# oswsnqc/Tensorflow-DPPO

Measured on AMD Instinct MI355X. Metric: env-steps/sec (whole node), Humanoid-shaped MLP DPPO at 1/2/4/8 MI355X, higher is better.
Workload: dtype fp32; 1 GPU; model=Humanoid-v4 MLP 64x64 tanh, preset=humanoid, global_batch=16777216, num_envs_per_gpu=262144, rollout_T=64, update_steps=4, parallelism=dp1

## Files before the change

dppo_amd/ops/hip/bindings.cpp:

```cpp
#include <torch/extension.h>

#include <vector>

std::vector<torch::Tensor> gae_scan(torch::Tensor rewards, torch::Tensor values,
                                    torch::Tensor dones, torch::Tensor boot,
                                    double gamma, double lam, bool whiten,
                                    double eps, torch::Tensor adv_out,
                                    torch::Tensor etr_out);

torch::Tensor ppo_loss_gauss_fwd(torch::Tensor pdpi, torch::Tensor pdold,
                                 torch::Tensor vpred, torch::Tensor oldv,
                                 torch::Tensor act, torch::Tensor adv,
                                 torch::Tensor etr, double clip,
                                 double entcoeff, double vcoeff);

torch::Tensor ppo_loss_gauss_gh(torch::Tensor pdflat, torch::Tensor oldflat,
                                torch::Tensor vpred, torch::Tensor oldv,
                                torch::Tensor act, torch::Tensor adv,
                                torch::Tensor etr, double clip,
                                double entcoeff, double vcoeff,
                                torch::Tensor clip_dev);

std::vector<torch::Tensor> ppo_loss_gauss_bwd(
    torch::Tensor pdpi, torch::Tensor pdold, torch::Tensor vpred,
// ... 35 lines not shown
                   torch::Tensor adv, torch::Tensor etr, torch::Tensor gh,
                   torch::Tensor clip_dev, double clip, double entcoeff,
                   double vcoeff);

void adam_step(torch::Tensor p, torch::Tensor g, torch::Tensor m,
               torch::Tensor v, int64_t step, double lr, double beta1,
               double beta2, double eps);

void adam_step_dev(torch::Tensor p, torch::Tensor g, torch::Tensor m,
                   torch::Tensor v, torch::Tensor step_dev,
                   torch::Tensor lr_dev, torch::Tensor coef, double beta1,
                   double beta2, double eps);

void gemm_fwd(torch::Tensor X, torch::Tensor Wt, torch::Tensor bias,
              int64_t activation, int64_t heads, torch::Tensor C,
              torch::Tensor v, torch::Tensor aux, int64_t wt_layout,
              int64_t ablate, int64_t ldc);

void dw_mfma(torch::Tensor delta, torch::Tensor acts, torch::Tensor grad_buf,
             int64_t w_off, int64_t b_off, int64_t split_row, int64_t w_off2,
             int64_t b_off2, int64_t ablate);

void rollout_sample(torch::Tensor pdflat, torch::Tensor actions,
                    torch::Tensor xva, torch::Tensor seed_dev,
                    torch::Tensor eps_dev, int64_t step, int64_t va_off,
                    double act_low, double act_high);

void gemm_env_step(torch::Tensor xva, torch::Tensor M, torch::Tensor xin,
                   torch::Tensor xout, torch::Tensor envd,
                   torch::Tensor horizons, torch::Tensor t,
                   torch::Tensor epr,
                   torch::Tensor rewards, torch::Tensor dones,
                   torch::Tensor rsum, torch::Tensor seed_dev, double sigma,
                   int64_t step);

void rollout_env_step(torch::Tensor xin, torch::Tensor xout, torch::Tensor G,
                      torch::Tensor envd, torch::Tensor horizons,
                      torch::Tensor t, torch::Tensor epr,
                      torch::Tensor rewards, torch::Tensor dones,
                      torch::Tensor seed_dev, double sigma, int64_t step);

torch::Tensor rollout_moments(torch::Tensor rewards, torch::Tensor dones,
                              torch::Tensor epr_in, int64_t T, int64_t E);

bool mlp_chunk_supported(int64_t D, int64_t H, int64_t A, int64_t n_hidden);

void mlp_chunk_train(
    torch::Tensor params, torch::Tensor states, torch::Tensor actions,
    torch::Tensor adv, torch::Tensor etr, torch::Tensor oldflat,
    torch::Tensor oldv, std::vector<int64_t> offsets,
    std::vector<int64_t> dims, int64_t activation, torch::Tensor clip_dev,
    double clip, double entcoeff, double vcoeff, torch::Tensor slabs,
    torch::Tensor mom, torch::Tensor vel, torch::Tensor step_dev,
    torch::Tensor lr_dev, torch::Tensor coef, torch::Tensor flat_grad,
    bool fuse_adam, double beta1, double beta2, double eps);

std::vector<torch::Tensor> rollout_run(
    torch::Tensor params, std::vector<int64_t> offsets,
    std::vector<int64_t> dims, int64_t activation,
    torch::Tensor envblob, int64_t rank, torch::Tensor horizons,
    double noise, double act_low, double act_high, double eps_explore,
    torch::Tensor x, torch::Tensor t, torch::Tensor epr,
    int64_t T, int64_t act_dim, int64_t seed, torch::Tensor out_buf,
    int64_t ablate);

PYBIND11_MODULE(TORCH_EXTENSION_NAME, mod) {
  mod.def("gae_scan", &gae_scan,
          "segmented GAE reverse scan + whitening (gfx950)");
  mod.def("ppo_loss_gauss_fwd", &ppo_loss_gauss_fwd,
          "fused DiagGaussian PPO loss forward (gfx950)");
  mod.def("ppo_loss_gauss_bwd", &ppo_loss_gauss_bwd,
          "fused DiagGaussian PPO loss backward (gfx950)");
  mod.def("ppo_loss_cat_fwd", &ppo_loss_cat_fwd,
          "fused Categorical PPO loss forward (gfx950)");
  mod.def("ppo_loss_cat_bwd", &ppo_loss_cat_bwd,
          "fused Categorical PPO loss backward (gfx950)");
  mod.def("cat_sample", &cat_sample,
          "Gumbel-max categorical sampling, counter-based RNG (gfx950)");
  mod.def("bf16_mm256", &bf16_mm256,
          "bf16 MFMA GEMM, 256^2 tile, pipelined glds, fused epilogues "
          "(gfx950)");
  mod.def("bf16_mm_small", &bf16_mm_small,
          "guarded bf16 MFMA GEMM for ragged heads shapes (gfx950)");
  mod.def("bf16_transpose", &bf16_transpose,
          "bf16 2D transpose with fused column sums (gfx950)");
  mod.def("gauss_gh_wide", &gauss_gh_wide,
          "wide-policy PPO loss gradient -> bf16 [g_pd | g_v] (gfx950)");
  mod.def("adam_step", &adam_step, "fused flat Adam step (gfx950)");
  mod.def("adam_step_dev", &adam_step_dev,
          "graph-replayable fused Adam (device step/lr) (gfx950)");
  mod.def("rollout_run", &rollout_run,
          "fused T-step rollout: MLP fwd + sample + synthetic env (gfx950)");
  mod.def("rollout_sample", &rollout_sample,
          "per-step action sampling + eps-greedy (v3 rollout) (gfx950)");
  mod.def("gemm_env_step", &gemm_env_step,
          "fused G-GEMM + env transition epilogue + per-env finish "
          "(v3 rollout; gfx950)");
  mod.def("rollout_env_step", &rollout_env_step,
          "per-step synthetic env finish: tanh/reward/done/reset (gfx950)");
  mod.def("rollout_moments", &rollout_moments,
          "episode-reward moments from reward/done streams (gfx950)");
  mod.def("ppo_loss_gauss_gh", &ppo_loss_gauss_gh,
          "wave-per-row PPO loss gradient -> [g_pd | g_v] (gfx950)");
  mod.def("gemm_fwd", &gemm_fwd,
          "MFMA f32 layer forward C=act(X@Wt+b), fused tanh (gfx950)");
  mod.def("dw_mfma", &dw_mfma,
          "MFMA f32 split-K dW += delta^T@acts into flat grad (gfx950)");
  mod.def("mlp_chunk_supported", &mlp_chunk_supported,
          "shape eligibility for the fused chunk-step kernel (gfx950)");
  mod.def("mlp_chunk_train", &mlp_chunk_train,
          "fused small-MLP training chunk step: fwd+PPO grad+bwd+dW "
          "partials + slab-reduce Adam (gfx950)");
}
```

dppo_amd/ops/hip/common.h:

```cpp
#pragma once

#include <hip/hip_runtime.h>

#define DEV_INLINE __device__ __forceinline__

constexpr int WAVE = 64;
constexpr int N_CU = 256;

DEV_INLINE float wave_reduce_sum(float x) {
  #pragma unroll
  for (int off = WAVE / 2; off > 0; off >>= 1) x += __shfl_down(x, off, WAVE);
  return x;
}

DEV_INLINE void wave_atomic_add(double* dst, float val) {
  float w = wave_reduce_sum(val);
  if ((threadIdx.x & (WAVE - 1)) == 0) atomicAdd(dst, static_cast<double>(w));
}

DEV_INLINE float fast_tanhf(float x) {
  const float e = __expf(2.0f * x);
  return 1.0f - 2.0f / (e + 1.0f);
}

DEV_INLINE int64_t gidx() {
  return static_cast<int64_t>(blockIdx.x) * blockDim.x + threadIdx.x;
}

DEV_INLINE int64_t gstride() {
  return static_cast<int64_t>(gridDim.x) * blockDim.x;
}

inline int elementwise_grid(int64_t n, int block) {
  int64_t g = (n + block - 1) / block;
  const int64_t cap = 2048;
  return static_cast<int>(g < cap ? (g > 0 ? g : 1) : cap);
}
```

dppo_amd/ops/hip/mfma_gemm.hip:

```cpp

#include <hip/hip_runtime.h>
#include <torch/extension.h>
#include <c10/hip/HIPStream.h>

#include "common.h"

namespace {

using f32x16 = __attribute__((ext_vector_type(16))) float;

constexpr int BK = 16;
constexpr int M_WAVE = 32;
constexpr int FWD_WAVES = 4;
constexpr int FWD_M = FWD_WAVES * M_WAVE;
constexpr int MAX_NT = 4;

DEV_INLINE int cd_row(int reg, int lane) {
  return (reg & 3) + 8 * (reg >> 2) + 4 * (lane >> 5);
}


struct FwdArgs {
  const float* X;
  const float* Wt;
  const float* bias;
  const float* aux;
  float* C;
  float* v;
  int64_t B;
  int K, N;
  int activation;
  int heads;
  int wt_layout;
  int ldc;
  int ablate;
  const float* env_xin;
  float* env_x;
  const float* envd;
  const int* horizons;
  const int* tcount;
  const long long* seed_dev;
  float* env_rsum;
  float sigma;
  int step;
};

DEV_INLINE unsigned g_lowbias32(unsigned x) {
  x ^= x >> 16;
  x *= 0x7feb352dU;
  x ^= x >> 15;
  x *= 0x846ca68bU;
  x ^= x >> 16;
  return x;
}
DEV_INLINE float2 g_rng_normal2(unsigned seed, int env, int step, int slot) {
  const unsigned h = g_lowbias32(seed ^ (unsigned)env * 0x9E3779B9U ^
                                 (unsigned)step * 0x85EBCA6BU ^
                                 (unsigned)slot * 0xC2B2AE35U);
  const float u1 = ((h >> 16) + 1) * (1.0f / 65537.0f);
  const float u2 = (h & 0xFFFFu) * (1.0f / 65536.0f);
  const float r = sqrtf(-2.0f * __logf(u1));
  float sn, cs;
  __sincosf(6.2831853071795865f * u2, &sn, &cs);
  return make_float2(r * cs, r * sn);
}
DEV_INLINE float g_rng_normal(unsigned seed, int env, int step, int slot) {
  return g_rng_normal2(seed, env, step, slot).x;
}

template <int NT>
__launch_bounds__(FWD_WAVES * 64)
__global__ void gemm_fwd_kernel(FwdArgs a) {
  const int lane = threadIdx.x & (WAVE - 1);
  const int wave = threadIdx.x / WAVE;

// ... 266 lines not shown
      if (col < a.N) {
        const float bv = (a.activation >= 3) ? 0.f : a.bias[col];
        #pragma unroll
        for (int r = 0; r < 16; ++r) {
          const int64_t row = b0 + wave * M_WAVE + cd_row(r, lane);
          if (row < a.B) {
            float x;
            if (a.activation >= 3) {
              const float h = a.aux[row * a.N + col];
              x = acc[t][r] * ((a.activation == 3) ? (1.f - h * h)
                                                   : (h > 0.f ? 1.f : 0.f));
            } else {
              x = acc[t][r] + bv;
              if (a.activation == 0) x = fmaxf(x, 0.f);
              else if (a.activation == 1) x = fast_tanhf(x);
            }
            if (a.heads == 2) {
              if (col == a.N - 2) a.v[row] = x;
              else if (col < a.N - 2) a.C[row * a.ldc + col] = x;
            } else if (a.heads) {
              if (col == a.N - 1) a.v[row] = x;
              else a.C[row * a.ldc + col] = x;
            } else {
              a.C[row * a.ldc + col] = x;
            }
          }
        }
      }
    }
  }
}


template <int RING>
__launch_bounds__(FWD_WAVES * 64, RING == 2 ? 6 : RING == 3 ? 4 : 3)
__global__ void gemm_fwd_glds_kernel(FwdArgs a) {
  constexpr int NT = 2;
  constexpr int PBK = 16;
  constexpr int NW = NT * M_WAVE;
  constexpr int XB = FWD_M * PBK * 4;
  constexpr int WB = PBK * NW * 4;
  constexpr int SLOT = XB + WB;
  __shared__ __attribute__((aligned(16))) char smem[RING * SLOT];
  const int tid = threadIdx.x;
  const int lane = tid & (WAVE - 1);
  const int wave = tid / WAVE;
  const int i_l = lane & 31;
  const int k_l = lane >> 5;
  const int n0 = blockIdx.y * NW;

  const int64_t b0 = (int64_t)blockIdx.x * FWD_M;
  if (b0 >= a.B) return;

  const float* srcX[2];
  int xcol[2];
  int64_t xrow[2];
  #pragma unroll
  for (int p = 0; p < 2; ++p) {
    const int q = tid + p * FWD_WAVES * 64;
    const int r = q >> 2;
    const int c4 = (q & 3) ^ (r & 3);
    int64_t row = b0 + r;
    row = row < a.B ? row : a.B - 1;
    xrow[p] = row;
    xcol[p] = c4 * 4;
    srcX[p] = a.X + row * a.K;
  }
// ... 45 lines not shown
    const int rem = min(S - 1 - s, RING - 2);
    if (rem >= RING - 2)
      asm volatile("s_waitcnt vmcnt(%0)" ::"i"(3 * (RING - 2)) : "memory");
    else if (RING == 4 && rem == 1)
      asm volatile("s_waitcnt vmcnt(3)" ::: "memory");
    else
      asm volatile("s_waitcnt vmcnt(0)" ::: "memory");
    __builtin_amdgcn_s_barrier();
    char* slot = smem + (s % RING) * SLOT;
    float* xs = (float*)slot;
    float* ws = (float*)(slot + XB);
    const int kb = smap(s) * PBK;
    if (kb + PBK > a.K) {
      for (int idx = tid; idx < (kb + PBK - a.K) * NW; idx += FWD_WAVES * 64)
        ws[(a.K - kb) * NW + idx] = 0.f;
      __builtin_amdgcn_s_barrier();
    }
    if (s + RING - 1 < S) issue(s + RING - 1);
    #pragma unroll 4
    for (int k2 = 0; k2 < PBK; k2 += 2) {
      const int k = k2 + k_l;
      const int row = wave * M_WAVE + i_l;
      const float av = xs[row * PBK + (((k >> 2) ^ (row & 3)) << 2) + (k & 3)];
      #pragma unroll
      for (int t = 0; t < NT; ++t) {
        const float bv = ws[k * NW + t * M_WAVE + i_l];
        acc[t] = __builtin_amdgcn_mfma_f32_32x32x2f32(av, bv, acc[t], 0, 0, 0);
      }
    }
  }
  asm volatile("s_waitcnt vmcnt(0)" ::: "memory");
  __builtin_amdgcn_s_barrier();

  if (a.activation == 5) {
    const unsigned seed = (unsigned)(*a.seed_dev);
    #pragma unroll
    for (int r = 0; r < 16; ++r) {
      const int64_t row = b0 + wave * M_WAVE + cd_row(r, lane);
      const bool rok = row < a.B;
      const int done =
          rok ? (a.tcount[row] + 1 >= a.horizons[row] ? 1 : 0) : 0;
      float part = 0.f;
      #pragma unroll
      for (int t = 0; t < NT; ++t) {
        const int col = n0 + t * M_WAVE + i_l;
        if (rok && col < a.N) {
          const float dv = a.envd[col];
          const float xv = a.env_xin[row * a.N + col];
          float nz = 0.f;
          if (a.sigma != 0.f) {
            const float2 pr =
                g_rng_normal2(seed, (int)row, a.step, 1000 + (col >> 1));
            nz = (col & 1) ? pr.y : pr.x;
          }
          const float pred = fast_tanhf(xv * dv + acc[t][r] + a.sigma * nz);
          part += pred * pred;
          const float out =
              done ? 0.1f * g_rng_normal(seed, (int)row, a.step, 5000 + col)
                   : pred;
          a.env_x[row * a.N + col] = out;
        }
      }
      #pragma unroll
      for (int off = 16; off > 0; off >>= 1)
        part += __shfl_down(part, off, 32);
      if (i_l == 0 && rok)
        a.env_rsum[(int64_t)blockIdx.y * a.B + row] = part;
    }
    return;
  }

  #pragma unroll
  for (int t = 0; t < NT; ++t) {
    const int col = n0 + t * M_WAVE + i_l;
    if (col < a.N) {
      const float bv = (a.activation >= 3) ? 0.f : a.bias[col];
      #pragma unroll
      for (int r = 0; r < 16; ++r) {
        const int64_t row = b0 + wave * M_WAVE + cd_row(r, lane);
        if (row < a.B) {
          float x;
          if (a.activation >= 3) {
            const float h = a.aux[row * a.N + col];
            x = acc[t][r] * ((a.activation == 3) ? (1.f - h * h)
                                                 : (h > 0.f ? 1.f : 0.f));
          } else {
            x = acc[t][r] + bv;
            if (a.activation == 0) x = fmaxf(x, 0.f);
            else if (a.activation == 1) x = fast_tanhf(x);
          }
          if (a.heads == 2) {
            if (col == a.N - 2) a.v[row] = x;
            else if (col < a.N - 2) a.C[row * a.ldc + col] = x;
          } else if (a.heads) {
            if (col == a.N - 1) a.v[row] = x;
            else a.C[row * a.ldc + col] = x;
          } else {
            a.C[row * a.ldc + col] = x;
          }
        }
      }
    }
  }
}

__global__ void env_finish2_kernel(const float* __restrict__ rsum,
                                   int* __restrict__ t,
                                   const int* __restrict__ horizons,
                                   float* __restrict__ epr,
                                   float* __restrict__ rewards,
                                   float* __restrict__ dones, int64_t E,
                                   int D, int npanels) {
  for (int64_t e = gidx(); e < E; e += gstride()) {
    float ss = 0.f;
    for (int p = 0; p < npanels; ++p) ss += rsum[(int64_t)p * E + e];
    const float r = 1.0f - ss / (float)D;
    rewards[e] = r;
    float ep = epr[e] + r;
    int tc = t[e] + 1;
    const int done = tc >= horizons[e] ? 1 : 0;
    dones[e] = (float)done;
    if (done) {
      ep = 0.f;
      tc = 0;
    }
    epr[e] = ep;
    t[e] = tc;
  }
}


struct DwArgs {
  const float* delta;
  const float* acts;
  float* slab;
  float* db_slab;
  int64_t B;
  int out_dim, in_dim;
  int nt;
  int splits;
  int ablate;
};

template <int NT, int MT>
__launch_bounds__(64, (NT == 2 && MT == 2) ? 3 : 1)
__global__ void dw_mfma_kernel(DwArgs a) {
  const int lane = threadIdx.x;
  const int m0 = blockIdx.x * (M_WAVE * MT);
  const int n_base = blockIdx.y * a.nt * M_WAVE;
  const int split = blockIdx.z;

  const int64_t rows_per = (a.B + a.splits - 1) / a.splits;
  const int64_t k0 = split * rows_per;
  const int64_t k1 = min(a.B, k0 + rows_per);

  const int i_l = lane & 31;
  const int k_l = lane >> 5;
  int mcol[MT];
  bool m_ok[MT];
  #pragma unroll
// ... 267 lines not shown
  const int s1 = min(splits, s0 + DW_RED_CHUNK);
  for (int64_t i = (int64_t)blockIdx.x * blockDim.x + threadIdx.x; i < n;
       i += (int64_t)gridDim.x * blockDim.x) {
    float acc = 0.f;
    for (int s = s0; s < s1; ++s) acc += slab[(int64_t)s * n + i];
    const int64_t mrow = i / in_dim;
    float* dst = (split_row >= 0 && mrow >= split_row)
                     ? &dW2[(mrow - split_row) * in_dim + i % in_dim]
                     : &dW[i];
    atomicAdd(dst, acc);
  }
}

__global__ void db_reduce_kernel(const float* __restrict__ db_slab,
                                 float* __restrict__ db,
                                 float* __restrict__ db2, int64_t out_dim,
                                 int splits, int split_row) {
  const int m = blockIdx.x;
  if (m >= out_dim) return;
  const int lane = threadIdx.x;
  float acc = 0.f;
  for (int s = lane; s < splits; s += WAVE)
    acc += db_slab[(int64_t)s * out_dim + m];
  acc = wave_reduce_sum(acc);
  if (lane == 0) {
    if (split_row >= 0 && m >= split_row) db2[m - split_row] += acc;
    else if (db != nullptr) db[m] += acc;
  }
}

}


void gemm_fwd(torch::Tensor X, torch::Tensor Wt, torch::Tensor bias,
              int64_t activation, int64_t heads, torch::Tensor C,
              torch::Tensor v, torch::Tensor aux, int64_t wt_layout,
              int64_t ablate, int64_t ldc) {
  const int64_t B = X.size(0);
  const int K = static_cast<int>(X.size(1));
  const int N = static_cast<int>(wt_layout ? Wt.size(0) : Wt.size(1));
  TORCH_CHECK(X.is_cuda() && X.is_contiguous() && Wt.is_contiguous());
  TORCH_CHECK(C.is_contiguous());
  TORCH_CHECK((wt_layout ? Wt.size(1) : Wt.size(0)) == K);
  TORCH_CHECK(activation >= 3 || bias.numel() == N);
  const int ncols = static_cast<int>(heads == 2 ? N - 2 : heads ? N - 1 : N);
  const int ldc_eff = static_cast<int>(ldc > 0 ? ldc : ncols);
  TORCH_CHECK(ldc_eff >= ncols);
  if (heads) {
    TORCH_CHECK(C.numel() >= (B - 1) * ldc_eff + ncols && v.numel() == B);
  } else {
    TORCH_CHECK(C.numel() >= (B - 1) * ldc_eff + ncols);
  }

  FwdArgs a{};
  a.X = X.data_ptr<float>();
  a.Wt = Wt.data_ptr<float>();
  a.bias = bias.data_ptr<float>();
  a.B = B;
  a.K = K;
  a.N = N;
  a.activation = static_cast<int>(activation);
  a.heads = static_cast<int>(heads);
  a.wt_layout = static_cast<int>(wt_layout);
  a.ablate = static_cast<int>(ablate);
  a.ldc = ldc_eff;
  a.C = C.data_ptr<float>();
  a.v = heads ? v.data_ptr<float>() : nullptr;
  if (activation >= 3) {
    TORCH_CHECK(aux.numel() == B * N, "dgrad mode needs aux = fwd activations");
    a.aux = aux.data_ptr<float>();
  }

  hipStream_t stream = c10::hip::getCurrentHIPStream().stream();
  const int64_t tiles = (B + FWD_M - 1) / FWD_M;
  const int grid = static_cast<int>(std::min<int64_t>(tiles, 4096));
  const int grid_pipe = static_cast<int>(std::min<int64_t>(tiles, 1 << 22));
  const int NT = (N + M_WAVE - 1) / M_WAVE;
  static const int pipe_env = []() {
    const char* e = getenv("DPPO_GEMM_PIPE");
    return e ? atoi(e) : 1;
  }();
  static const int pbk_env = []() {
    const char* e = getenv("DPPO_GEMM_PBK");
    return e ? atoi(e) : 0;
  }();
  const bool pipe = pipe_env && !a.ablate && K >= 4 &&
                    (K % 4 == 0 || (wt_layout == 0 && activation >= 3)) &&
                    (wt_layout == 1 || (N >= 4 && N % 4 == 0));
  const int pbk = pbk_env ? pbk_env : 16;
  static const int glds_env = []() {
    const char* e = getenv("DPPO_GEMM_GLDS");
    return e ? atoi(e) : 1;
  }();
  const bool glds_ok = glds_env && !a.ablate && wt_layout == 0 &&
                       K % 4 == 0 && K >= 4 && N % 4 == 0 && N >= 4 &&
                       a.activation != 9999;
  static const int ring_env = []() {
    const char* e = getenv("DPPO_FWD_RING");
    return e ? atoi(e) : 0;
  }();
  const int ring_sel = ring_env ? ring_env : (a.K <= 128 ? 2 : 3);
  #define DISPATCH_FWD(NTV, NPANEL)                                          \
    if (glds_ok && NTV == 2 && ring_sel == 2)                                \
      hipLaunchKernelGGL(gemm_fwd_glds_kernel<2>,                            \
                         dim3((unsigned)grid_pipe, NPANEL),                  \
                         dim3(FWD_WAVES * 64), 0, stream, a);                \
    else if (glds_ok && NTV == 2 && ring_sel == 4)                           \
      hipLaunchKernelGGL(gemm_fwd_glds_kernel<4>,                            \
                         dim3((unsigned)grid_pipe, NPANEL),                  \
                         dim3(FWD_WAVES * 64), 0, stream, a);                \
    else if (glds_ok && NTV == 2)                                            \
      hipLaunchKernelGGL(gemm_fwd_glds_kernel<3>,                            \
                         dim3((unsigned)grid_pipe, NPANEL),                  \
                         dim3(FWD_WAVES * 64), 0, stream, a);                \
    else if (pipe && pbk == 32)                                              \
      hipLaunchKernelGGL((gemm_fwd_pipe_kernel<NTV, 32>),                    \
                         dim3(grid_pipe, NPANEL), dim3(FWD_WAVES * 64), 0,   \
                         stream, a);                                         \
    else if (pipe)                                                           \
      hipLaunchKernelGGL((gemm_fwd_pipe_kernel<NTV, 16>),                    \
                         dim3(grid_pipe, NPANEL), dim3(FWD_WAVES * 64), 0,   \
                         stream, a);                                         \
    else                                                                     \
      hipLaunchKernelGGL(gemm_fwd_kernel<NTV>, dim3(grid),                   \
                         dim3(FWD_WAVES * 64), 0, stream, a)
  if (N > MAX_NT * M_WAVE) {
    TORCH_CHECK(pipe, "N > 128 needs the pipelined path (K%4==0 etc.)");
    const int panels = (N + 2 * M_WAVE - 1) / (2 * M_WAVE);
    DISPATCH_FWD(2, panels);
  } else {
    switch (NT) {
      case 1: DISPATCH_FWD(1, 1); break;
      case 2: DISPATCH_FWD(2, 1); break;
      case 3: DISPATCH_FWD(3, 1); break;
      default: DISPATCH_FWD(4, 1); break;
    }
  }
  #undef DISPATCH_FWD
}

void gemm_env_step(torch::Tensor xva, torch::Tensor M, torch::Tensor xin,
                   torch::Tensor xout, torch::Tensor envd,
                   torch::Tensor horizons, torch::Tensor t,
                   torch::Tensor epr,
                   torch::Tensor rewards, torch::Tensor dones,
                   torch::Tensor rsum, torch::Tensor seed_dev, double sigma,
                   int64_t step) {
  const int64_t E = xva.size(0);
  const int K = static_cast<int>(xva.size(1));
  const int D = static_cast<int>(M.size(1));
  TORCH_CHECK(xva.is_contiguous() && M.is_contiguous() &&
              xin.is_contiguous() && xout.is_contiguous());
  TORCH_CHECK(M.size(0) == K && xin.size(0) == E && xin.size(1) == D);
  TORCH_CHECK(xout.numel() == E * D);
  TORCH_CHECK(K % 4 == 0 && D % 4 == 0, "fused env step needs 16B rows");
  TORCH_CHECK(horizons.dtype() == torch::kInt32 && t.dtype() == torch::kInt32);
  const int panels_chk = (D + 63) / 64;
  TORCH_CHECK(rsum.numel() >= panels_chk * E);
  FwdArgs a{};
  a.X = xva.data_ptr<float>();
  a.Wt = M.data_ptr<float>();
  a.B = E;
  a.K = K;
  a.N = D;
  a.activation = 5;
  a.ldc = D;
  a.env_xin = xin.data_ptr<float>();
  a.env_x = xout.data_ptr<float>();
  a.envd = envd.data_ptr<float>();
  a.horizons = horizons.data_ptr<int>();
  a.tcount = t.data_ptr<int>();
  a.seed_dev = reinterpret_cast<const long long*>(seed_dev.data_ptr<int64_t>());
  a.env_rsum = rsum.data_ptr<float>();
  a.sigma = (float)sigma;
  a.step = (int)step;
  hipStream_t stream = c10::hip::getCurrentHIPStream().stream();
  const int64_t tiles = (E + FWD_M - 1) / FWD_M;
  const int panels = (D + 63) / 64;
  hipLaunchKernelGGL(gemm_fwd_glds_kernel<3>,
                     dim3((unsigned)tiles, (unsigned)panels),
                     dim3(FWD_WAVES * 64), 0, stream, a);
  hipLaunchKernelGGL(env_finish2_kernel, dim3(elementwise_grid(E, 256)),
                     dim3(256), 0, stream, rsum.data_ptr<float>(),
                     t.data_ptr<int>(), horizons.data_ptr<int>(),
                     epr.data_ptr<float>(), rewards.data_ptr<float>(),
                     dones.data_ptr<float>(), E, D, panels);
}

static torch::Tensor& dw_scratch(int idx, int64_t need,
                                 const torch::TensorOptions& opt) {
  static torch::Tensor cache[2];
  static std::vector<torch::Tensor> retired;
  torch::Tensor& t = cache[idx];
  if (!t.defined() || t.numel() < need) {
    if (t.defined()) retired.push_back(t);
    t = torch::empty({need}, opt);
  }
  return t;
}

void dw_mfma(torch::Tensor delta, torch::Tensor acts, torch::Tensor grad_buf,
             int64_t w_off, int64_t b_off, int64_t split_row, int64_t w_off2,
             int64_t b_off2, int64_t ablate) {
  const int64_t B = delta.size(0);
  const int out_dim = static_cast<int>(delta.size(1));
  const int in_dim = static_cast<int>(acts.size(1));
  TORCH_CHECK(delta.is_contiguous() && acts.is_contiguous());

  DwArgs a{};
  a.delta = delta.data_ptr<float>();
  a.acts = acts.data_ptr<float>();
  a.B = B;
  a.out_dim = out_dim;
  a.in_dim = in_dim;
  a.ablate = static_cast<int>(ablate);
  const int mt = (out_dim >= 64) ? 2 : 1;
  a.nt = std::min(mt == 2 ? 2 : MAX_NT, (in_dim + M_WAVE - 1) / M_WAVE);
  const int m_tiles = (out_dim + M_WAVE * mt - 1) / (M_WAVE * mt);
  const int n_tiles = (in_dim + a.nt * M_WAVE - 1) / (a.nt * M_WAVE);
// ... 92 lines not shown
```

dppo_amd/ops/hip/rollout.hip:

```cpp

#include <hip/hip_runtime.h>
#include <torch/extension.h>
#include <c10/hip/HIPStream.h>

#include "common.h"

namespace {

constexpr int ENV_TILE = 8;
constexpr int MAX_D = 512;
constexpr int MAX_H = 128;
constexpr int MAX_A = 32;
constexpr int MAX_R = 32;
constexpr int MAX_HIDDEN = 3;

constexpr int NWAVES = 4;

struct LdsMap {
  int x, h0, h1, pd, act, xv, part, val, rsum, epr, racc;
  int xs, hs, total;
};

DEV_INLINE LdsMap lds_map(int D, int Hmax, int A, int rank, int et) {
  auto r4 = [](int v) { return (v + 3) & ~3; };
// ... 484 lines not shown
    const float logstd = pdflat[e * P + A + j];
    float act = mean + __expf(logstd) * rng_normal(seed, (int)e, step, j);
    const float u_dec = rng_uniform(seed, (int)e, step, 90001);
    if (u_dec < eps) {
      const float u = rng_uniform(seed, (int)e, step, 90010 + j);
      act = act_low + (act_high - act_low) * u;
    }
    actions[e * A + j] = act;
    xva[e * xva_w + va_off + j] = act;
  }
}

__global__ void env_finish_kernel(
    const float* __restrict__ xin,
    float* __restrict__ xout,
    const float* __restrict__ G,
    const float* __restrict__ envd,
    const int* __restrict__ horizons,
    int* __restrict__ t,
    float* __restrict__ epr,
    float* __restrict__ rewards,
    float* __restrict__ dones,
    const long* __restrict__ seed_dev, float sigma, int step, int64_t E,
    int D) {
  const unsigned seed = (unsigned)*seed_dev;
  const int lane = threadIdx.x & (WAVE - 1);
  const int64_t wid =
      ((int64_t)blockIdx.x * blockDim.x + threadIdx.x) / WAVE;
  if (wid >= E) return;
  const int64_t e = wid;
  constexpr int CMAX = (MAX_D / 4 + WAVE - 1) / WAVE;
  const int nc4 = D / 4;
  float4 xn[CMAX];
  float ss = 0.f;
  int it = 0;
  for (int c = lane; c < nc4; c += WAVE, ++it) {
    const int d = 4 * c;
    const float4 xv = *reinterpret_cast<const float4*>(&xin[e * D + d]);
    const float4 gv = *reinterpret_cast<const float4*>(&G[e * D + d]);
    const float4 dv = *reinterpret_cast<const float4*>(&envd[d]);
    float nz[4] = {0.f, 0.f, 0.f, 0.f};
    if (sigma != 0.f) {
      const float2 p0 = rng_normal2(seed, (int)e, step, 1000 + 2 * c);
      const float2 p1 = rng_normal2(seed, (int)e, step, 1000 + 2 * c + 1);
      nz[0] = p0.x; nz[1] = p0.y; nz[2] = p1.x; nz[3] = p1.y;
    }
    float4 v;
    v.x = fast_tanhf(xv.x * dv.x + gv.x + sigma * nz[0]);
    v.y = fast_tanhf(xv.y * dv.y + gv.y + sigma * nz[1]);
    v.z = fast_tanhf(xv.z * dv.z + gv.z + sigma * nz[2]);
    v.w = fast_tanhf(xv.w * dv.w + gv.w + sigma * nz[3]);
    xn[it] = v;
    ss += v.x * v.x + v.y * v.y + v.z * v.z + v.w * v.w;
  }
  ss = wave_reduce_sum(ss);
  int done;
  if (lane == 0) {
    const float r = 1.0f - ss / D;
    rewards[e] = r;
    float ep = epr[e] + r;
    int tc = t[e] + 1;
    done = (tc >= horizons[e]) ? 1 : 0;
    dones[e] = (float)done;
    if (done) {
      ep = 0.f;
      tc = 0;
    }
    epr[e] = ep;
    t[e] = tc;
  }
  done = __shfl(done, 0, WAVE);
  it = 0;
  for (int c = lane; c < nc4; c += WAVE, ++it) {
    const int d = 4 * c;
    float4 v = xn[it];
    if (done) {
      v.x = 0.1f * rng_normal(seed, (int)e, step, 5000 + d);
      v.y = 0.1f * rng_normal(seed, (int)e, step, 5000 + d + 1);
      v.z = 0.1f * rng_normal(seed, (int)e, step, 5000 + d + 2);
      v.w = 0.1f * rng_normal(seed, (int)e, step, 5000 + d + 3);
    }
    *reinterpret_cast<float4*>(&xout[e * D + d]) = v;
  }
}

}

std::vector<torch::Tensor> rollout_run(
    torch::Tensor params, std::vector<int64_t> offsets,
    std::vector<int64_t> dims, int64_t activation,
    torch::Tensor envblob, int64_t rank, torch::Tensor horizons,
    double noise, double act_low, double act_high, double eps_explore,
    torch::Tensor x, torch::Tensor t, torch::Tensor epr,
    int64_t T, int64_t act_dim, int64_t seed, torch::Tensor out_buf,
    int64_t ablate) {
  const int64_t E = x.size(0);
  const int64_t D = x.size(1);
  const int A = static_cast<int>(act_dim);
  const int n_hidden = static_cast<int>(dims.size()) - 1;
  TORCH_CHECK(x.is_cuda() && x.dtype() == torch::kFloat32 && x.is_contiguous());
  TORCH_CHECK(params.is_contiguous() && params.dtype() == torch::kFloat32);
  TORCH_CHECK(n_hidden >= 1 && n_hidden <= MAX_HIDDEN, "1..3 hidden layers");
  TORCH_CHECK(D <= MAX_D && A <= MAX_A && rank <= MAX_R,
              "dims exceed rollout-kernel limits");
  TORCH_CHECK(dims[0] == D, "first layer must consume obs_dim");
  TORCH_CHECK(horizons.dtype() == torch::kInt32 && t.dtype() == torch::kInt32);
// ... 199 lines not shown
```

dppo_amd/trainer.py:

```python

from __future__ import annotations

import contextlib
import math
import os
from dataclasses import dataclass
from typing import Dict, Optional, Tuple

import torch

from .config import DPPOConfig, game_spaces
from .envs.synthetic import BatchedSyntheticEnv, make_env
from .models.mlp import PolicyValueMLP
from .ops import gae_advantages, ppo_losses, PPOLossCoeffs
from .parallel.comm import Comm, FlatBuffers
from .utils.logging import ScalarLogger
from .utils.timers import PhaseTimers
from . import spaces

STATS_DIM = 11


@dataclass
class RolloutBatch:
# ... 337 lines not shown
        E, T = c.NUM_ENVS, c.MAX_EPOCH_STEPS
        D = self.obs_space.shape[0]
        A = self.act_space.shape[0]
        P = 2 * A
        H = tuple(c.HIDDEN_SIZES)
        key = (E, T, D, A, H)
        if getattr(self, "_v3_key", None) == key:
            return self._v3
        dev = self.device
        r = env.rank_eff
        kw = ((r + A + 3) // 4) * 4
        M = torch.zeros(kw, D, device=dev)
        M[:r] = env.U
        M[r:r + A] = env.B
        B = int(E) * T
        self._v3 = dict(
            xva=torch.zeros(E, kw, device=dev), va_off=r, kw=kw,
            M=M.contiguous(), V=env.V.contiguous(),
            G=torch.empty(E, D, device=dev),
            h=[torch.empty(E, hh, device=dev) for hh in H],
            bz_r=torch.zeros(r, device=dev),
            bz_D=torch.zeros(D, device=dev),
            wh=torch.empty(P + 1, H[-1], device=dev),
            bh=torch.empty(P + 1, device=dev),
            whT_pad=(torch.zeros(H[-1], P + 2, device=dev)
                     if (P + 2) % 4 == 0
                     and os.environ.get("DPPO_HEADS_PAD") != "0" else None),
            bh_pad=torch.zeros(P + 2, device=dev),
            pd_scratch=torch.empty(E, P, device=dev),
            seed_dev=torch.zeros(1, dtype=torch.int64, device=dev),
            eps_dev=torch.zeros(1, dtype=torch.float32, device=dev),
            epr_before=torch.empty(E, device=dev),
            rsum=torch.zeros(((D + 63) // 64) * E, device=dev),
            empty=torch.empty(0, device=dev),
            acts=torch.empty(sum(B * hh for hh in H), device=dev),
        )
        self._v3_key = key
        return self._v3

    @staticmethod
    def _env_fused() -> bool:
        return os.environ.get("DPPO_ENV_FUSED") == "1"

    def _v3_body(self, states, pdflats, actions, values, rewards, dones,
                 boot_v):
        from .ops import hip_ext

        ext = hip_ext()
        c, env, v3 = self.cfg, self.env, self._v3
        E, T = c.NUM_ENVS, c.MAX_EPOCH_STEPS
        D = self.obs_space.shape[0]
        A = self.act_space.shape[0]
        P = 2 * A
        act_code = 1 if c.ACTIVATION == "tanh" else 0
        low = float(self.act_space.low.flat[0])
        high = float(self.act_space.high.flat[0])
        n_h = len(c.HIDDEN_SIZES)
        wh, bh = v3["wh"], v3["bh"]
        wh[:P].copy_(self.pi.pi.weight.detach())
        wh[P:].copy_(self.pi.vf.weight.detach())
        bh[:P].copy_(self.pi.pi.bias.detach())
        bh[P:].copy_(self.pi.vf.bias.detach())
        whT_pad = v3.get("whT_pad")
        if whT_pad is not None:
            whT_pad[:, :P + 1].copy_(wh.t())
            v3["bh_pad"][:P + 1].copy_(bh)
        wts = self._wt_bufs()
        for l, lay in enumerate(self.pi.hidden):
            wts[l].copy_(lay.weight.detach().t())
        v3["epr_before"].copy_(self.epr)
        states[0].reshape(-1).copy_(env.x.reshape(-1))
        hs = c.HIDDEN_SIZES
        B = T * E
        acts_views, off = [], 0
        for hh in hs:
            acts_views.append(v3["acts"].narrow(0, off, B * hh).view(B, hh))
            off += B * hh
        for st in range(T):
            xin = states[st]
            h = xin
            for l in range(n_h):
                hl = acts_views[l].narrow(0, st * E, E)
                ext.gemm_fwd(h, wts[l],
                             self.pi.hidden[l].bias.detach(), act_code, 0,
                             hl, hl, hl, 0, 0, 0)
                h = hl
            if whT_pad is not None:
                ext.gemm_fwd(h, whT_pad, v3["bh_pad"], 2, 2, pdflats[st],
                             values[st], pdflats[st], 0, 0, 0)
            else:
                ext.gemm_fwd(h, wh, bh, 2, 1, pdflats[st], values[st],
                             pdflats[st], 1, 0, 0)
            ext.gemm_fwd(xin, v3["V"], v3["bz_r"], 2, 0, v3["xva"],
                         v3["xva"], v3["xva"], 0, 0, v3["kw"])
            ext.rollout_sample(pdflats[st], actions[st], v3["xva"],
                               v3["seed_dev"], v3["eps_dev"], st,
                               v3["va_off"], low, high)
            xout = states[st + 1] if st + 1 < T else env.x
            if self._env_fused():
                ext.gemm_env_step(v3["xva"], v3["M"], xin, xout, env.d,
                                  env.horizons_i32, env.t, self.epr,
                                  rewards[st], dones[st], v3["rsum"],
                                  v3["seed_dev"], float(env.NOISE), st)
            else:
                ext.gemm_fwd(v3["xva"], v3["M"], v3["bz_D"], 2, 0, v3["G"],
                             v3["G"], v3["G"], 0, 0, 0)
                ext.rollout_env_step(xin, xout, v3["G"], env.d,
                                     env.horizons_i32, env.t, self.epr,
                                     rewards[st], dones[st], v3["seed_dev"],
                                     float(env.NOISE), st)
        h = env.x
        for l in range(n_h):
            hl = v3["h"][l]
            ext.gemm_fwd(h, wts[l],
                         self.pi.hidden[l].bias.detach(), act_code, 0,
                         hl, hl, hl, 0, 0, 0)
            h = hl
        if whT_pad is not None:
            ext.gemm_fwd(h, whT_pad, v3["bh_pad"], 2, 2, v3["pd_scratch"],
                         boot_v, v3["pd_scratch"], 0, 0, 0)
        else:
            ext.gemm_fwd(h, wh, bh, 2, 1, v3["pd_scratch"], boot_v,
                         v3["pd_scratch"], 1, 0, 0)
        return ext.rollout_moments(rewards, dones, v3["epr_before"], T, E)

    @torch.no_grad()
    def _rollout_once_hip_v3(self) -> Tuple[RolloutBatch, Dict[str, float]]:
        c, E = self.cfg, self.cfg.NUM_ENVS
        T = c.MAX_EPOCH_STEPS
        eps = self.exploration_rate()
        env = self.env
        self._rollout_counter = getattr(self, "_rollout_counter", 0) + 1
        seed = (
            c.SEED * 1_000_003
            + self.comm.rank * 7_919
            + self._rollout_counter * 104_729
# ... 918 lines not shown
```

Before: 93.32 million env-steps/s.

## Make fused env step the default and vectorize its epilogue with optional x@V fold

Makes the fused G-GEMM + env-transition kernel the default path (DPPO_ENV_FUSED now defaults on) and rewrites its epilogue. Accumulators are staged through swizzled LDS so each lane handles float4 columns, with vectorized loads/stores and a 16-lane shuffle reduction. It also adds an opt-in (default off) fold that computes the next step's x@V inside the epilogue via MFMA, plus a per-panel reduce kernel. The ring size for the env kernel now follows the shared selector, and the unfused env-step kernel gets a panel-ordered sum so its reward reduction matches the fused path. The default switch removes a separate G GEMM launch and its round-trip through memory, at the cost of extra LDS traffic and register pressure.

Measured after the change: 100.6 million env-steps/s (median of 6 runs). +7.9%, better.

```diff
diff --git a/dppo_amd/ops/hip/bindings.cpp b/dppo_amd/ops/hip/bindings.cpp
--- a/dppo_amd/ops/hip/bindings.cpp
+++ b/dppo_amd/ops/hip/bindings.cpp
@@ -91,7 +91,7 @@
                    torch::Tensor epr,
                    torch::Tensor rewards, torch::Tensor dones,
                    torch::Tensor rsum, torch::Tensor seed_dev, double sigma,
-                   int64_t step);
+                   int64_t step, torch::Tensor V, torch::Tensor xvp);
 
 void rollout_env_step(torch::Tensor xin, torch::Tensor xout, torch::Tensor G,
                       torch::Tensor envd, torch::Tensor horizons,
@@ -153,8 +153,8 @@
   mod.def("rollout_sample", &rollout_sample,
           "per-step action sampling + eps-greedy (v3 rollout) (gfx950)");
   mod.def("gemm_env_step", &gemm_env_step,
-          "fused G-GEMM + env transition epilogue + per-env finish "
-          "(v3 rollout; gfx950)");
+          "fused G-GEMM + env transition epilogue + per-env finish, "
+          "optionally folding the next step's x@V (v3 rollout; gfx950)");
   mod.def("rollout_env_step", &rollout_env_step,
           "per-step synthetic env finish: tanh/reward/done/reset (gfx950)");
   mod.def("rollout_moments", &rollout_moments,
diff --git a/dppo_amd/ops/hip/common.h b/dppo_amd/ops/hip/common.h
--- a/dppo_amd/ops/hip/common.h
+++ b/dppo_amd/ops/hip/common.h
@@ -23,6 +23,11 @@
   return 1.0f - 2.0f / (e + 1.0f);
 }
 
+DEV_INLINE float sq4(float4 v) {
+  return __fmaf_rn(v.w, v.w,
+                   __fmaf_rn(v.z, v.z, __fmaf_rn(v.y, v.y, __fmul_rn(v.x, v.x))));
+}
+
 DEV_INLINE int64_t gidx() {
   return static_cast<int64_t>(blockIdx.x) * blockDim.x + threadIdx.x;
 }
diff --git a/dppo_amd/ops/hip/mfma_gemm.hip b/dppo_amd/ops/hip/mfma_gemm.hip
--- a/dppo_amd/ops/hip/mfma_gemm.hip
+++ b/dppo_amd/ops/hip/mfma_gemm.hip
@@ -8,6 +8,7 @@
 namespace {
 
 using f32x16 = __attribute__((ext_vector_type(16))) float;
+using f32x4 = __attribute__((ext_vector_type(4))) float;
 
 constexpr int BK = 16;
 constexpr int M_WAVE = 32;
@@ -41,6 +42,8 @@
   const int* tcount;
   const long long* seed_dev;
   float* env_rsum;
+  const float* env_V;
+  float* env_xvp;
   float sigma;
   int step;
 };
@@ -373,7 +376,8 @@
 }
 
 
-template <int RING>
+template <int RING,
+          bool ENV = false>
 __launch_bounds__(FWD_WAVES * 64, RING == 2 ? 6 : RING == 3 ? 4 : 3)
 __global__ void gemm_fwd_glds_kernel(FwdArgs a) {
   constexpr int NT = 2;
@@ -485,40 +489,111 @@
   asm volatile("s_waitcnt vmcnt(0)" ::: "memory");
   __builtin_amdgcn_s_barrier();
 
-  if (a.activation == 5) {
+  if constexpr (ENV) {
+    constexpr int HR = 16;
+    static_assert(RING * SLOT >= FWD_WAVES * HR * NW * 4 + NW * 16 * 4,
+                  "env epilogue image + V panel must fit the ring");
+    float* tile = reinterpret_cast<float*>(smem) + wave * (HR * NW);
+    float* vs = reinterpret_cast<float*>(smem) + FWD_WAVES * HR * NW;
+    const bool fold = a.env_xvp != nullptr;
+    if (fold) {
+      const int kl = tid >> 2;
+      const int kr = n0 + kl;
+      float4 vv = make_float4(0.f, 0.f, 0.f, 0.f);
+      if (kr < a.N)
+        vv = *reinterpret_cast<const float4*>(
+            &a.env_V[(int64_t)kr * 16 + 4 * (tid & 3)]);
+      *reinterpret_cast<float4*>(
+          &vs[(kl ^ ((kl >> 2) & 1)) * 16 + 4 * (tid & 3)]) = vv;
+      __syncthreads();
+    }
     const unsigned seed = (unsigned)(*a.seed_dev);
-    #pragma unroll
-    for (int r = 0; r < 16; ++r) {
-      const int64_t row = b0 + wave * M_WAVE + cd_row(r, lane);
-      const bool rok = row < a.B;
-      const int done =
-          rok ? (a.tcount[row] + 1 >= a.horizons[row] ? 1 : 0) : 0;
-      float part = 0.f;
+    const float sigma = a.sigma;
+    const int step = a.step;
+    const int c4 = lane & 15;
+    const int rsub = lane >> 4;
+    const int d = n0 + 4 * c4;
+    const int c = d >> 2;
+    const bool cok = d < a.N;
+    float4 dv = make_float4(0.f, 0.f, 0.f, 0.f);
+    if (cok) dv = *reinterpret_cast<const float4*>(&a.envd[d]);
+    #pragma unroll
+    for (int h = 0; h < 2; ++h) {
+      int ln = lane;
+      asm volatile("" : "+v"(ln));
       #pragma unroll
       for (int t = 0; t < NT; ++t) {
-        const int col = n0 + t * M_WAVE + i_l;
-        if (rok && col < a.N) {
-          const float dv = a.envd[col];
-          const float xv = a.env_xin[row * a.N + col];
-          float nz = 0.f;
-          if (a.sigma != 0.f) {
-            const float2 pr =
-                g_rng_normal2(seed, (int)row, a.step, 1000 + (col >> 1));
-            nz = (col & 1) ? pr.y : pr.x;
+        #pragma unroll
+        for (int q = 0; q < 8; ++q) {
+          const int lr = cd_row(8 * h + q, ln) - HR * h;
+          const int cc = t * M_WAVE + (ln & 31);
+          tile[lr * NW + ((((cc >> 2) ^ lr) << 2) | (cc & 3))] =
+              acc[t][8 * h + q];
+        }
+      }
+      asm volatile("s_waitcnt lgkmcnt(0)" ::: "memory");
+      #pragma unroll
+      for (int j = 0; j < 4; ++j) {
+        const int lr = 4 * j + rsub;
+        const int64_t e = b0 + wave * M_WAVE + HR * h + lr;
+        const bool rok = e < a.B;
+        float4* slot =
+            reinterpret_cast<float4*>(&tile[lr * NW + ((c4 ^ lr) << 2)]);
+        float4 v = make_float4(0.f, 0.f, 0.f, 0.f);
+        float ss = 0.f;
+        if (rok && cok) {
+          const float4 gv = *slot;
+          const float4 xv =
+              *reinterpret_cast<const float4*>(&a.env_xin[e * a.N + d]);
+          float nz[4] = {0.f, 0.f, 0.f, 0.f};
+          if (sigma != 0.f) {
+            const float2 p0 = g_rng_normal2(seed, (int)e, step, 1000 + 2 * c);
+            const float2 p1 =
+                g_rng_normal2(seed, (int)e, step, 1000 + 2 * c + 1);
+            nz[0] = p0.x; nz[1] = p0.y; nz[2] = p1.x; nz[3] = p1.y;
           }
-          const float pred = fast_tanhf(xv * dv + acc[t][r] + a.sigma * nz);
-          part += pred * pred;
-          const float out =
-              done ? 0.1f * g_rng_normal(seed, (int)row, a.step, 5000 + col)
-                   : pred;
-          a.env_x[row * a.N + col] = out;
+          v.x = fast_tanhf(xv.x * dv.x + gv.x + sigma * nz[0]);
+          v.y = fast_tanhf(xv.y * dv.y + gv.y + sigma * nz[1]);
+          v.z = fast_tanhf(xv.z * dv.z + gv.z + sigma * nz[2]);
+          v.w = fast_tanhf(xv.w * dv.w + gv.w + sigma * nz[3]);
+          ss = sq4(v);
+          const int done = a.tcount[e] + 1 >= a.horizons[e] ? 1 : 0;
+          if (done) {
+            v.x = 0.1f * g_rng_normal(seed, (int)e, step, 5000 + d);
+            v.y = 0.1f * g_rng_normal(seed, (int)e, step, 5000 + d + 1);
+            v.z = 0.1f * g_rng_normal(seed, (int)e, step, 5000 + d + 2);
+            v.w = 0.1f * g_rng_normal(seed, (int)e, step, 5000 + d + 3);
+          }
+          *reinterpret_cast<float4*>(&a.env_x[e * a.N + d]) = v;
         }
-      }
-      #pragma unroll
-      for (int off = 16; off > 0; off >>= 1)
-        part += __shfl_down(part, off, 32);
-      if (i_l == 0 && rok)
-        a.env_rsum[(int64_t)blockIdx.y * a.B + row] = part;
+        #pragma unroll
+        for (int off = 8; off > 0; off >>= 1) ss += __shfl_xor(ss, off, 16);
+        if (c4 == 0 && rok) a.env_rsum[(int64_t)blockIdx.y * a.B + e] = ss;
+        if (fold) *slot = v;
+      }
+      if (fold) {
+        asm volatile("s_waitcnt lgkmcnt(0)" ::: "memory");
+        const int fi = lane & 15;
+        f32x4 xa = {0.f, 0.f, 0.f, 0.f};
+        #pragma unroll
+        for (int q = 0; q < 4; ++q) {
+          const float4 av = *reinterpret_cast<const float4*>(
+              &tile[fi * NW + (((4 * q + rsub) ^ fi) << 2)]);
+          const float am[4] = {av.x, av.y, av.z, av.w};
+          #pragma unroll
+          for (int m = 0; m < 4; ++m) {
+            const int k = 4 * (4 * q + rsub) + m;
+            const float bv = vs[(k ^ ((k >> 2) & 1)) * 16 + fi];
+            xa = __builtin_amdgcn_mfma_f32_16x16x4f32(am[m], bv, xa, 0, 0, 0);
+          }
+        }
+        #pragma unroll
+        for (int r = 0; r < 4; ++r) {
+          const int64_t e = b0 + wave * M_WAVE + HR * h + 4 * rsub + r;
+          if (e < a.B)
+            a.env_xvp[((int64_t)blockIdx.y * a.B + e) * 16 + fi] = xa[r];
+        }
+      }
     }
     return;
   }
@@ -579,6 +654,22 @@
     }
     epr[e] = ep;
     t[e] = tc;
+  }
+}
+
+__global__ void env_xv_reduce_kernel(const float* __restrict__ xvp,
+                                     float* __restrict__ xva, int64_t E,
+                                     int kw, int npanels) {
+  for (int64_t i = gidx(); i < E * 4; i += gstride()) {
+    const int64_t e = i >> 2;
+    const int q = (int)(i & 3);
+    float4 s = make_float4(0.f, 0.f, 0.f, 0.f);
+    for (int p = 0; p < npanels; ++p) {
+      const float4 v = *reinterpret_cast<const float4*>(
+          &xvp[((int64_t)p * E + e) * 16 + 4 * q]);
+      s.x += v.x; s.y += v.y; s.z += v.z; s.w += v.w;
+    }
+    *reinterpret_cast<float4*>(&xva[e * kw + 4 * q]) = s;
   }
 }
 
@@ -912,6 +1003,14 @@
 }
 
 
+static int fwd_ring_for(int K) {
+  static const int ring_env = []() {
+    const char* e = getenv("DPPO_FWD_RING");
+    return e ? atoi(e) : 0;
+  }();
+  return ring_env ? ring_env : (K <= 128 ? 2 : 3);
+}
+
 void gemm_fwd(torch::Tensor X, torch::Tensor Wt, torch::Tensor bias,
               int64_t activation, int64_t heads, torch::Tensor C,
               torch::Tensor v, torch::Tensor aux, int64_t wt_layout,
@@ -975,11 +1074,7 @@
   const bool glds_ok = glds_env && !a.ablate && wt_layout == 0 &&
                        K % 4 == 0 && K >= 4 && N % 4 == 0 && N >= 4 &&
                        a.activation != 9999;
-  static const int ring_env = []() {
-    const char* e = getenv("DPPO_FWD_RING");
-    return e ? atoi(e) : 0;
-  }();
-  const int ring_sel = ring_env ? ring_env : (a.K <= 128 ? 2 : 3);
+  const int ring_sel = fwd_ring_for(a.K);
   #define DISPATCH_FWD(NTV, NPANEL)                                          \
     if (glds_ok && NTV == 2 && ring_sel == 2)                                \
       hipLaunchKernelGGL(gemm_fwd_glds_kernel<2>,                            \
@@ -1025,7 +1120,7 @@
                    torch::Tensor epr,
                    torch::Tensor rewards, torch::Tensor dones,
                    torch::Tensor rsum, torch::Tensor seed_dev, double sigma,
-                   int64_t step) {
+                   int64_t step, torch::Tensor V, torch::Tensor xvp) {
   const int64_t E = xva.size(0);
   const int K = static_cast<int>(xva.size(1));
   const int D = static_cast<int>(M.size(1));
@@ -1054,17 +1149,43 @@
   a.env_rsum = rsum.data_ptr<float>();
   a.sigma = (float)sigma;
   a.step = (int)step;
+  const int panels = (D + 63) / 64;
+  const bool fold = xvp.numel() > 0;
+  if (fold) {
+    TORCH_CHECK(V.is_contiguous() && V.dim() == 2 && V.size(0) == D &&
+                    V.size(1) == 16,
+                "x@V fold needs V = [D][16]");
+    TORCH_CHECK(K >= 16 && xvp.is_contiguous() &&
+                xvp.numel() >= (int64_t)panels * E * 16);
+    a.env_V = V.data_ptr<float>();
+    a.env_xvp = xvp.data_ptr<float>();
+  }
   hipStream_t stream = c10::hip::getCurrentHIPStream().stream();
   const int64_t tiles = (E + FWD_M - 1) / FWD_M;
-  const int panels = (D + 63) / 64;
-  hipLaunchKernelGGL(gemm_fwd_glds_kernel<3>,
-                     dim3((unsigned)tiles, (unsigned)panels),
-                     dim3(FWD_WAVES * 64), 0, stream, a);
+  const dim3 grid((unsigned)tiles, (unsigned)panels);
+  switch (fwd_ring_for(K)) {
+    case 2:
+      hipLaunchKernelGGL((gemm_fwd_glds_kernel<2, true>), grid,
+                         dim3(FWD_WAVES * 64), 0, stream, a);
+      break;
+    case 4:
+      hipLaunchKernelGGL((gemm_fwd_glds_kernel<4, true>), grid,
+                         dim3(FWD_WAVES * 64), 0, stream, a);
+      break;
+    default:
+      hipLaunchKernelGGL((gemm_fwd_glds_kernel<3, true>), grid,
+                         dim3(FWD_WAVES * 64), 0, stream, a);
+  }
   hipLaunchKernelGGL(env_finish2_kernel, dim3(elementwise_grid(E, 256)),
                      dim3(256), 0, stream, rsum.data_ptr<float>(),
                      t.data_ptr<int>(), horizons.data_ptr<int>(),
                      epr.data_ptr<float>(), rewards.data_ptr<float>(),
                      dones.data_ptr<float>(), E, D, panels);
+  if (fold)
+    hipLaunchKernelGGL(env_xv_reduce_kernel,
+                       dim3(elementwise_grid(E * 4, 256)), dim3(256), 0,
+                       stream, xvp.data_ptr<float>(), xva.data_ptr<float>(),
+                       E, K, panels);
 }
 
 static torch::Tensor& dw_scratch(int idx, int64_t need,
diff --git a/dppo_amd/ops/hip/rollout.hip b/dppo_amd/ops/hip/rollout.hip
--- a/dppo_amd/ops/hip/rollout.hip
+++ b/dppo_amd/ops/hip/rollout.hip
@@ -540,28 +540,44 @@
   constexpr int CMAX = (MAX_D / 4 + WAVE - 1) / WAVE;
   const int nc4 = D / 4;
   float4 xn[CMAX];
+  float pp[CMAX];
+  #pragma unroll
+  for (int it = 0; it < CMAX; ++it) {
+    const int c = lane + it * WAVE;
+    float ps = 0.f;
+    if (c < nc4) {
+      const int d = 4 * c;
+      const float4 xv = *reinterpret_cast<const float4*>(&xin[e * D + d]);
+      const float4 gv = *reinterpret_cast<const float4*>(&G[e * D + d]);
+      const float4 dv = *reinterpret_cast<const float4*>(&envd[d]);
+      float nz[4] = {0.f, 0.f, 0.f, 0.f};
+      if (sigma != 0.f) {
+        const float2 p0 = rng_normal2(seed, (int)e, step, 1000 + 2 * c);
+        const float2 p1 = rng_normal2(seed, (int)e, step, 1000 + 2 * c + 1);
+        nz[0] = p0.x; nz[1] = p0.y; nz[2] = p1.x; nz[3] = p1.y;
+      }
+      float4 v;
+      v.x = fast_tanhf(xv.x * dv.x + gv.x + sigma * nz[0]);
+      v.y = fast_tanhf(xv.y * dv.y + gv.y + sigma * nz[1]);
+      v.z = fast_tanhf(xv.z * dv.z + gv.z + sigma * nz[2]);
+      v.w = fast_tanhf(xv.w * dv.w + gv.w + sigma * nz[3]);
+      xn[it] = v;
+      ps = sq4(v);
+    }
+    #pragma unroll
+    for (int off = 8; off > 0; off >>= 1) ps += __shfl_xor(ps, off, 16);
+    pp[it] = ps;
+  }
   float ss = 0.f;
-  int it = 0;
-  for (int c = lane; c < nc4; c += WAVE, ++it) {
-    const int d = 4 * c;
-    const float4 xv = *reinterpret_cast<const float4*>(&xin[e * D + d]);
-    const float4 gv = *reinterpret_cast<const float4*>(&G[e * D + d]);
-    const float4 dv = *reinterpret_cast<const float4*>(&envd[d]);
-    float nz[4] = {0.f, 0.f, 0.f, 0.f};
-    if (sigma != 0.f) {
-      const float2 p0 = rng_normal2(seed, (int)e, step, 1000 + 2 * c);
-      const float2 p1 = rng_normal2(seed, (int)e, step, 1000 + 2 * c + 1);
-      nz[0] = p0.x; nz[1] = p0.y; nz[2] = p1.x; nz[3] = p1.y;
-    }
-    float4 v;
-    v.x = fast_tanhf(xv.x * dv.x + gv.x + sigma * nz[0]);
-    v.y = fast_tanhf(xv.y * dv.y + gv.y + sigma * nz[1]);
-    v.z = fast_tanhf(xv.z * dv.z + gv.z + sigma * nz[2]);
-    v.w = fast_tanhf(xv.w * dv.w + gv.w + sigma * nz[3]);
-    xn[it] = v;
-    ss += v.x * v.x + v.y * v.y + v.z * v.z + v.w * v.w;
-  }
-  ss = wave_reduce_sum(ss);
+  const int npanels = (D + 63) / 64;
+  #pragma unroll
+  for (int it = 0; it < CMAX; ++it) {
+    #pragma unroll
+    for (int g = 0; g < 4; ++g) {
+      const float part = __shfl(pp[it], g * 16, WAVE);
+      if (4 * it + g < npanels) ss += part;
+    }
+  }
   int done;
   if (lane == 0) {
     const float r = 1.0f - ss / D;
@@ -578,8 +594,10 @@
     t[e] = tc;
   }
   done = __shfl(done, 0, WAVE);
-  it = 0;
-  for (int c = lane; c < nc4; c += WAVE, ++it) {
+  #pragma unroll
+  for (int it = 0; it < CMAX; ++it) {
+    const int c = lane + it * WAVE;
+    if (c >= nc4) break;
     const int d = 4 * c;
     float4 v = xn[it];
     if (done) {
diff --git a/dppo_amd/trainer.py b/dppo_amd/trainer.py
--- a/dppo_amd/trainer.py
+++ b/dppo_amd/trainer.py
@@ -393,6 +393,8 @@
             eps_dev=torch.zeros(1, dtype=torch.float32, device=dev),
             epr_before=torch.empty(E, device=dev),
             rsum=torch.zeros(((D + 63) // 64) * E, device=dev),
+            xvp=(torch.empty(((D + 63) // 64) * E * 16, device=dev)
+                 if r == 16 else None),
             empty=torch.empty(0, device=dev),
             acts=torch.empty(sum(B * hh for hh in H), device=dev),
         )
@@ -401,7 +403,11 @@
 
     @staticmethod
     def _env_fused() -> bool:
-        return os.environ.get("DPPO_ENV_FUSED") == "1"
+        return os.environ.get("DPPO_ENV_FUSED", "1") != "0"
+
+    @staticmethod
+    def _xv_fold() -> bool:
+        return os.environ.get("DPPO_XV_FOLD", "0") == "1"
 
     def _v3_body(self, states, pdflats, actions, values, rewards, dones,
                  boot_v):
@@ -437,6 +443,9 @@
         for hh in hs:
             acts_views.append(v3["acts"].narrow(0, off, B * hh).view(B, hh))
             off += B * hh
+        fused = self._env_fused()
+        fold = fused and self._xv_fold() and v3["xvp"] is not None
+        no_fold = (v3["empty"], v3["empty"])
         for st in range(T):
             xin = states[st]
             h = xin
@@ -452,17 +461,20 @@
             else:
                 ext.gemm_fwd(h, wh, bh, 2, 1, pdflats[st], values[st],
                              pdflats[st], 1, 0, 0)
-            ext.gemm_fwd(xin, v3["V"], v3["bz_r"], 2, 0, v3["xva"],
-                         v3["xva"], v3["xva"], 0, 0, v3["kw"])
+            if not fold or st == 0:
+                ext.gemm_fwd(xin, v3["V"], v3["bz_r"], 2, 0, v3["xva"],
+                             v3["xva"], v3["xva"], 0, 0, v3["kw"])
             ext.rollout_sample(pdflats[st], actions[st], v3["xva"],
                                v3["seed_dev"], v3["eps_dev"], st,
                                v3["va_off"], low, high)
             xout = states[st + 1] if st + 1 < T else env.x
-            if self._env_fused():
+            if fused:
                 ext.gemm_env_step(v3["xva"], v3["M"], xin, xout, env.d,
                                   env.horizons_i32, env.t, self.epr,
                                   rewards[st], dones[st], v3["rsum"],
-                                  v3["seed_dev"], float(env.NOISE), st)
+                                  v3["seed_dev"], float(env.NOISE), st,
+                                  *((v3["V"], v3["xvp"]) if fold
+                                    else no_fold))
             else:
                 ext.gemm_fwd(v3["xva"], v3["M"], v3["bz_D"], 2, 0, v3["G"],
                              v3["G"], v3["G"], 0, 0, 0)
```
